# singhhp1069/charon

Measured on AMD Instinct MI355X. Metric: verified+aggregated 3-of-4 threshold BLS sigs/sec at 1/2/4/8 MI355X, higher is better.
Workload: dtype u32 (Fp 14x28-bit limbs); 1 GPU; config2: 3-of-4, 10000 DVs x 1 attestation per GPU; parallelism=shard1, inflight_launches=3, batches_per_launch=16, rlc_group=16, rlc_chunk=8, gident=0, subgroup_batch=0, level0=passed, hw_queues=4

## Files before the change

### charon_amd/_native.py

```python
from __future__ import annotations

import ctypes
import os
import shutil
import subprocess

PKG = os.path.dirname(os.path.abspath(__file__))
ROOT = os.path.dirname(PKG)
CSRC = os.path.join(PKG, "csrc")
LIB_PATH = os.path.join(PKG, "libtbls_gpu.so")
HEADER = os.path.join(ROOT, "include", "tbls_gpu.h")
HEADERS = [HEADER, os.path.join(ROOT, "include", "tbls_ssz.h")]


def _hipcc():
    for c in ("/opt/rocm/bin/hipcc", shutil.which("hipcc") or ""):
        if c and os.path.exists(c):
            return c
    raise RuntimeError("hipcc not found: cannot build libtbls_gpu.so")


def _clangxx():
    c = "/opt/rocm/llvm/bin/clang++"
    if not os.path.exists(c):
# ... 158 lines not shown
        ("slots", ctypes.c_uint32),
        ("verify_mode", ctypes.c_uint32),
        ("rlc_group", ctypes.c_uint32),
        ("rlc_seed", ctypes.c_uint64),
        ("rlc_chunk", ctypes.c_uint32),
        ("streams_per_slot", ctypes.c_uint32),
        ("rlc_batch", ctypes.c_uint32),
        ("gident", ctypes.c_uint32),
        ("fb_window", ctypes.c_uint32),
        ("subgroup_batch", ctypes.c_uint32),
        ("express_partials", ctypes.c_uint32),
        ("l0_duty_partials", ctypes.c_uint32),
        ("l0_msg_share", ctypes.c_uint32),
        ("sgb_tri_partials", ctypes.c_uint32),
        ("sgb_tri_m", ctypes.c_uint32),
    ]


SIGNATURES = {
    "tbg_init": (ctypes.c_int, [ctypes.POINTER(TbgConfig), ctypes.POINTER(ctypes.c_void_p)]),
    "tbg_destroy": (None, [ctypes.c_void_p]),
    "tbg_strerror": (ctypes.c_char_p, [ctypes.c_int]),
    "tbg_device_count": (ctypes.c_int, []),
    "tbg_device_cu_count": (ctypes.c_int, [ctypes.c_int]),
    "tbg_synchronize": (ctypes.c_int, [ctypes.c_void_p]),
    "tbg_load_pubkeys": (ctypes.c_int, [ctypes.c_void_p, ctypes.c_void_p, ctypes.c_uint32,
                                        ctypes.POINTER(ctypes.c_uint32), ctypes.c_void_p]),
    "tbg_pubkey_count": (ctypes.c_uint32, [ctypes.c_void_p]),
    "tbg_submit": (ctypes.c_int, [ctypes.c_void_p, ctypes.POINTER(TbgBatch), ctypes.POINTER(ctypes.c_uint64)]),
    "tbg_collect": (ctypes.c_int, [ctypes.c_void_p, ctypes.c_uint64, ctypes.c_void_p, ctypes.c_void_p,
# ... 79 lines not shown
```

### charon_amd/csrc/k_msm.hip

```cpp
#define TBG_ADD_DBL_INLINE 1
#ifndef TBG_SCHED_FENCE
#define TBG_SCHED_FENCE 1
#endif
#include "tbls_launch.h"
#include "bls_msm.h"
#include "bls_pair.h"
#include "bls_batchinv.h"

namespace tbg {

__global__ void __launch_bounds__(BINV_BLOCK) k_pubkey_tables(const G1A* pk, const G1A* xpk, const int32_t* status,
                                                              uint32_t n, G1A* tab) {
  const uint32_t i = blockIdx.x * blockDim.x + threadIdx.x;
  const bool in = i < n;
  const bool ok = in && status[i] == DEC_OK;
  G1A p0{fp_zero(), fp_zero()}, x0 = p0;
  if (ok) {
    p0 = pk[i];
    x0 = xpk[i];
  }
#pragma unroll 1
  for (int k = 0; k < (int)PK_TAB; ++k) {
    const G1J e = ok ? rlc_key_table_w2_entry(p0, x0, k) : jac_inf<Fp>();
    G1A a{fp_zero(), fp_zero()};
    const bool got = block_jac_to_aff<BINV_WAVES>(e, ok, a);
    if (in) tab[(size_t)PK_TAB * i + k] = got ? a : G1A{fp_zero(), fp_zero()};
  }
}

__global__ void TBG_LAUNCH k_rlc_g1_l0(DevBatch B, const G1A* tab, const int32_t* pk_status, uint32_t n_pk) {
  const uint32_t i = blockIdx.x * blockDim.x + threadIdx.x;
  if (i >= B.n_partials || B.partial_status[i] != TBG_PS_NOT_VERIFIED) return;
  const uint32_t pid = B.pubkey_ids[i];
  const bool fused = l0_fused(B);
  if (pid >= n_pk || pk_status[pid] != DEC_OK) {
    B.partial_status[i] = TBG_PS_ERR_PUBKEY;
    if (fused) B.counters[CNT_L0_BAD] = 1;
    return;
  }
  if (fused) {
    const uint4 v = *(const uint4*)(B.l0f_u + 4ull * i);
    const uint32_t uf[4] = {v.x, v.y, v.z, v.w};
    B.part_p[i] = rlc_mul_key_l0f(tab + (size_t)PK_TAB * pid, fp_from_const(G1_BETA), uf);
    return;
  }
  const uint64_t r = rlc_scalar(B.rlc_seed, i);
  uint32_t u[4];
  rlc_digits(r, u);
  B.msm_r[i] = r;
  B.part_p[i] = rlc_mul_key(tab + (size_t)PK_TAB * pid, u);
#pragma unroll
  for (int k = 0; k < 4; ++k) {
    bool neg;
    atomicAdd(&B.msm_off[msm_bucket(u[k], neg)], 1u);
  }
}

namespace l0duty {
static_assert(BINV_BLOCK == kBlock, "k_rlc_g1_l0: the workgroup of the batched inversion");
__global__ void TBG_LAUNCH k_rlc_g1_l0(DevBatch B, const G1A* tab, const int32_t* pk_status, uint32_t n_pk) {
  const uint32_t d = blockIdx.x * blockDim.x + threadIdx.x;
  const bool in = d < B.n_duties;
  uint32_t i0 = 0, n = 0, cand = 0;
  if (in) {
    i0 = B.duty_first[d];
    n = B.duty_first[d + 1] - i0;
    for (uint32_t k = 0; k < n; ++k) {
      const uint32_t i = i0 + k;
      if (B.partial_status[i] != TBG_PS_NOT_VERIFIED) continue;
      const uint32_t pid = B.pubkey_ids[i];
      if (pid >= n_pk || pk_status[pid] != DEC_OK) {
        B.partial_status[i] = TBG_PS_ERR_PUBKEY;
        B.counters[CNT_L0_BAD] = 1;
        continue;
      }
      ++cand;
// ... 171 lines not shown
  __shared__ Jac<Fp2x> lds[2 * PAIRS];
  if (B.counters[CNT_L0_BAD]) return;
  const uint32_t pr = threadIdx.x >> 1;
  Jac<Fp2x> acc = jac_add_in<Fp2x, true>(px_load(B.msm_sum[2 * pr]), px_load(B.msm_sum[2 * pr + 1]));
  acc = pair_tree_sum<PAIRS>(acc, lds);
  if (pr != 0) return;
  if (jac_is_inf(acc)) {
    if (pair_par() == 0) B.counters[CNT_L0_BAD] = 1;
    return;
  }
  const Fp2x zi = f_inv(acc.Z);
  const Fp2x zi2 = f_sqr(zi);
  px_store(*B.batch_pt, Aff<Fp2x>{f_mul(acc.X, zi2), f_mul(acc.Y, f_mul(zi2, zi))});
}

__global__ void __launch_bounds__(2 * L0F_PAIRS) k_l0f_reduce(DevBatch B, uint32_t n_sg, uint32_t wq, uint32_t n_t) {
  __shared__ Jac<Fp2x> lds[2 * L0F_PAIRS];
  if (B.counters[CNT_L0_BAD]) return;
  const uint32_t pr = threadIdx.x >> 1, b = blockIdx.x;
  const bool qcol = b < SGB_K * wq;
  const uint32_t col = qcol ? b / wq : SGB_K, chunk = qcol ? b % wq : b - SGB_K * wq;
  const uint32_t count = qcol ? n_sg : n_sg * n_t;
  const uint32_t a0 = chunk * L0F_CHUNK + pr * L0F_PER, a1 = min(a0 + L0F_PER, count);
  Jac<Fp2x> acc = jac_inf<Fp2x>();
#pragma unroll 1
  for (uint32_t a = a0; a < a1; ++a) {
    if (qcol) {
      acc = jac_add_in<Fp2x, true>(acc, px_load(B.sgb_part[sgb_q_slot(B, a, col)]));
    } else {
      acc = jac_add_in<Fp2x, true>(acc, px_load(B.sgb_t[a]));
    }
  }
  acc = pair_tree_sum<L0F_PAIRS>(acc, lds);
  if (pr == 0) px_store(B.l0f_sum[b], acc);
}

__global__ void __launch_bounds__(2 * L0F_PAIRS) k_l0f_fold(DevBatch B, uint32_t wq, uint32_t wt) {
  TBG_URGENT();
  __shared__ Jac<Fp2x> lds[2 * L0F_PAIRS];
  if (B.counters[CNT_L0_BAD]) return;
  const uint32_t pr = threadIdx.x >> 1, col = blockIdx.x;
  const uint32_t first = col < SGB_K ? col * wq : SGB_K * wq, count = col < SGB_K ? wq : wt;
  Jac<Fp2x> acc = jac_inf<Fp2x>();
#pragma unroll 1
  for (uint32_t a = pr; a < count; a += L0F_PAIRS) acc = jac_add_in<Fp2x, true>(acc, px_load(B.l0f_sum[first + a]));
  acc = pair_tree_sum<L0F_PAIRS>(acc, lds);
  if (pr == 0) px_store(B.l0f_sum[SGB_K * wq + wt + col], acc);
}

constexpr uint32_t L0F_HORNER_THREADS = 8;
__global__ void __launch_bounds__(64) k_l0f_horner(DevBatch B, uint32_t base) {
  TBG_URGENT();
  __shared__ Jac<Fp2x> lds[L0F_HORNER_THREADS];
  if (B.counters[CNT_L0_BAD]) return;
  const int j = (int)(threadIdx.x >> 1);
  const G2J* tot = B.l0f_sum + base;
  const int e0 = l0f_first(j), e1 = l0f_first(j + 1);
  Jac<Fp2x> acc = px_load(tot[e1 - 1]);
#pragma unroll 1
  for (int e = e1 - 2; e >= e0; --e) acc = l0f_mul13_add(acc, px_load(tot[e]));
  acc = l0f_term(acc, px_load(tot[SGB_K]), j);
// ... 2 lines not shown
  if (jac_is_inf(acc)) {
    if (pair_par() == 0) B.counters[CNT_L0_BAD] = 1;
    return;
  }
  const Fp2x zi = f_inv(acc.Z);
  const Fp2x zi2 = f_sqr(zi);
  px_store(*B.batch_pt, Aff<Fp2x>{f_mul(acc.X, zi2), f_mul(acc.Y, f_mul(zi2, zi))});
}

void launch_pubkey_tables(const G1A* pk, const G1A* xpk, const int32_t* status, uint32_t n, G1A* tab, hipStream_t st) {
  if (n) TBG_KLAUNCH(k_pubkey_tables, dim3((n + BINV_BLOCK - 1) / BINV_BLOCK), dim3(BINV_BLOCK), st, pk, xpk, status, n,
                     tab);
}

void launch_l0_keys(const DevBatch& B, const G1A* pk_tab, const int32_t* pk_status, uint32_t n_pk, hipStream_t st) {
  if (l0_per_duty(B)) {
    using l0duty::k_rlc_g1_l0;
    TBG_KLAUNCH(k_rlc_g1_l0, grid_for(B.n_duties), dim3(kBlock), st, B, pk_tab, pk_status, n_pk);
    return;
  }
  if (B.n_partials) TBG_KLAUNCH(k_rlc_g1_l0, grid_for(B.n_partials), dim3(kBlock), st, B, pk_tab, pk_status, n_pk);
}

void launch_l0_msm(const DevBatch& B, hipStream_t st) {
  TBG_KLAUNCH(k_msm_scan, dim3(1), dim3(kScanBlock), st, B);
  if (B.n_partials) TBG_KLAUNCH(k_msm_scatter, grid_for(B.n_partials), dim3(kBlock), st, B);
  TBG_KLAUNCH(k_msm_bucket_part, grid_for(2 * MSM_BUCKETS * MSM_SPLIT), dim3(kBlock), st, B);
  TBG_KLAUNCH(k_msm_bucket, grid_for(2 * MSM_BUCKETS), dim3(kBlock), st, B);
  TBG_KLAUNCH(k_msm_tree, dim3(MSM_TREE_WG), dim3(2 * MSM_TREE_PAIRS), st, B);
  TBG_KLAUNCH(k_msm_tree_final, dim3(1), dim3(MSM_TREE_WG), st, B);
}

void launch_l0_fused_s(const DevBatch& B, hipStream_t st) {
  const uint32_t n_sg = sgb_groups(B.n_partials, B.sgb_m), n_t = sgb_t_slices(B.sgb_m);
  const uint32_t wq = l0f_q_chunks(n_sg), wt = l0f_t_chunks(n_sg, B.sgb_m);
  TBG_KLAUNCH(k_l0f_reduce, dim3(SGB_K * wq + wt), dim3(2 * L0F_PAIRS), st, B, n_sg, wq, n_t);
  TBG_KLAUNCH(k_l0f_fold, dim3(L0F_COLS), dim3(2 * L0F_PAIRS), st, B, wq, wt);
  TBG_KLAUNCH(k_l0f_horner, dim3(1), dim3(L0F_HORNER_THREADS), st, B, SGB_K * wq + wt);
}

}
```

### charon_amd/csrc/k_rlc.hip

```cpp
#define TBG_ADD_DBL_INLINE 1
#ifndef TBG_SCHED_FENCE
#define TBG_SCHED_FENCE 1
#endif
#include "tbls_launch.h"
#include "bls_h2c.h"
#include "bls_lines.h"
#include "bls_hex.h"
#include "bls_rlc.h"
#include "bls_batchinv.h"
#include "bls_row.h"

namespace tbg {

__device__ __forceinline__ bool rlc_usable(const DevBatch& B, uint32_t i, const int32_t* pk_status, uint32_t n_pk) {
  int32_t st = B.partial_status[i];
  if (st != TBG_PS_NOT_VERIFIED && st != TBG_PS_ERR_PUBKEY) return false;
  uint32_t pid = B.pubkey_ids[i];
  return pid < n_pk && pk_status[pid] == DEC_OK;
}
__device__ __forceinline__ bool rlc_candidate(const DevBatch& B, uint32_t i) {
  return B.partial_status[i] == TBG_PS_NOT_VERIFIED;
}

__device__ __forceinline__ bool rlc_combinable(const DevBatch& B, uint32_t d) {
// ... 664 lines not shown
}

void launch_rlc_prepare(const DevBatch& B, const G1A* pk_aff, const G1A* pk_tab, const int32_t* pk_status,
                        uint32_t n_pk, hipStream_t st, void (*after_keys)(const DevBatch&, hipStream_t)) {
  if (B.sets) launch_set_init(B, st);
  if (!B.n_duties) return;
  if (B.rlc_group == 0) {
    if (B.n_partials) TBG_KLAUNCH(k_list_all_partials, grid_for(B.n_partials), dim3(kBlock), st, B, pk_status, n_pk);
    if (after_keys) after_keys(B, st);
    return;
  }
  uint32_t n_groups = (B.n_duties + B.rlc_group - 1) / B.rlc_group;
  if (B.rlc_batch) {
    launch_l0_keys(B, pk_tab, pk_status, n_pk, st);
    if (after_keys) after_keys(B, st);
    if (l0_fused(B)) launch_l0_fused_s(B, st);
    else launch_l0_msm(B, st);
    if (!l0_per_duty(B)) TBG_KLAUNCH(k_rlc_duty_sum<DSUM_L0_P>, duty_grid(B), dim3(BINV_BLOCK), st, B);
    if (l0_by_msg(B)) launch_l0m_sums(B, st);
    launch_l0_lines(B, st);
    return;
  }
  if (after_keys) after_keys(B, st);
  launch_rlc_g1(B, pk_tab, pk_aff, pk_status, n_pk, st);
  TBG_KLAUNCH(k_rlc_duty_sum<DSUM_P>, duty_grid(B), dim3(BINV_BLOCK), st, B);
  launch_gm_group_s(B, st);
  launch_lines_fold(B, FOLD_GROUPS, n_groups, st);
}

static void launch_narrowing(const DevBatch& B, const G1A* pk_aff, uint32_t n_groups, uint32_t nch, hipStream_t st) {
  TBG_KLAUNCH(k_rlc_resolve_groups, grid_for(B.n_duties), dim3(kBlock), st, B);
  launch_gm_failed_partials(B, pk_aff, st);
// ... 84 lines not shown
```

### charon_amd/csrc/tbls_engine.hip

```cpp
#include <hip/hip_runtime.h>
#include <cstdio>
#include <cstdlib>
#include <cstring>
#include <cmath>
#include <functional>
#include <algorithm>
#include <atomic>
#include <chrono>
#include <mutex>
#include <new>
#include <random>
#include <thread>
#include <vector>
#include "tbls_launch.h"
#include "bls_l0msg.h"
#include "bls_lines.h"

using namespace tbg;

namespace tbg {
void debug_after_launch(const char* kernel, hipStream_t st) {
  static const bool on = getenv("TBG_DEBUG_SYNC") && getenv("TBG_DEBUG_SYNC")[0] == '1';
  if (!on) return;
  hipEvent_t a;
// ... 88 lines not shown
  tbg_ticket next_ticket = 1;
  float last_ms[8] = {};
  uint32_t rlc_group = 16;
  uint32_t rlc_chunk = 4;
  bool chunk_auto = true;
  bool rlc_auto = false;
  uint32_t rlc_batch = TBG_RLC_L0_AUTO;
  double invalid_ema = 0.0;
  uint64_t rlc_seed = 0;
  uint64_t seed_ctr = 0;
  uint32_t gident = TBG_GIDENT_OFF;
  uint32_t fb_window = TBG_FB_WINDOW;
  uint32_t sgb_mode = TBG_SGB_AUTO;
  uint32_t express_max = TBG_EXPRESS_PARTIALS;
  uint32_t l0_duty_partials = TBG_L0_DUTY_PARTIALS;
  uint32_t l0_msg_share = TBG_L0_MSG_SHARE;
  uint32_t sgb_tri_partials = TBG_SGB_TRI_PARTIALS;
  uint32_t sgb_tri_m = SGB_TRI_M;
  uint32_t n_simd = 1024;
  std::atomic<uint64_t> host[8] = {};
  double nonsub_ema = 0.0;
};

#define HIP_TRY(x)                       \
  do {                                   \
    hipError_t e_ = (x);                 \
    if (e_ != hipSuccess) return TBG_E_DEVICE; \
  } while (0)

static size_t arena_size(size_t need) {
// ... 83 lines not shown
  if (cfg && cfg->rlc_chunk) {
    c->rlc_chunk = cfg->rlc_chunk;
    c->chunk_auto = false;
  }
  if (c->rlc_group > 4096 || c->rlc_chunk > 4096) { delete c; return TBG_E_INVALID_ARG; }
  if (cfg && cfg->rlc_batch > TBG_RLC_L0_OFF) { delete c; return TBG_E_INVALID_ARG; }
  if (cfg) c->rlc_batch = cfg->rlc_batch;
  c->rlc_seed = cfg ? cfg->rlc_seed : 0;
  if (cfg && cfg->gident > TBG_GIDENT_CHUNKS) { delete c; return TBG_E_INVALID_ARG; }
  c->gident = cfg ? cfg->gident : (uint32_t)TBG_GIDENT_OFF;
  if (cfg && cfg->fb_window) c->fb_window = cfg->fb_window;
  if (cfg && cfg->subgroup_batch > TBG_SGB_OFF) { delete c; return TBG_E_INVALID_ARG; }
  if (cfg) c->sgb_mode = cfg->subgroup_batch;
  if (cfg && cfg->express_partials) c->express_max = cfg->express_partials;
  if (cfg && cfg->l0_duty_partials) c->l0_duty_partials = cfg->l0_duty_partials;
  if (cfg && cfg->l0_msg_share) c->l0_msg_share = cfg->l0_msg_share;
  if (cfg && cfg->sgb_tri_partials) c->sgb_tri_partials = cfg->sgb_tri_partials;
  if (cfg && cfg->sgb_tri_m) c->sgb_tri_m = cfg->sgb_tri_m;
  if (!sgb_triple(c->sgb_tri_m) || c->sgb_tri_m > SGB_TRI_M_MAX || (c->sgb_tri_m & (c->sgb_tri_m - 1))) {
    delete c;
    return TBG_E_INVALID_ARG;
  }
  if (hipSetDevice(dev) != hipSuccess || hipStreamCreateWithFlags(&c->stream, hipStreamNonBlocking) != hipSuccess ||
      hipEventCreateWithFlags(&c->retire_ev, hipEventDisableTiming) != hipSuccess ||
      hipEventCreateWithFlags(&c->keys_ready, hipEventDisableTiming) != hipSuccess) {
    if (c->retire_ev) hipEventDestroy(c->retire_ev);
    if (c->stream) hipStreamDestroy(c->stream);
    delete c;
    return TBG_E_DEVICE;
  }
// ... 742 lines not shown
  B.gm_hist = (uint32_t*)(dw + w_gmhist);
  B.gm_order = (uint32_t*)(dw + w_gmorder);
  B.sgb = sgb ? 1u : 0u;
  B.sgb_m = sgb_m;
  B.sgb_split = sgb_split;
  B.sgb_off = (uint32_t*)(dw + w_sgoff);
  B.sgb_ent = (uint32_t*)(dw + w_sgent);
  B.sgb_part = (G2J*)(dw + w_sgpart);
  B.sgb_rank = (uint32_t*)(dw + w_sgrank);
  B.sgb_code = (uint32_t*)(dw + w_sgcode);
  B.sgb_bad = (uint32_t*)(dw + w_sgbad);
  B.sgb_t = (G2J*)(dw + w_sgt);
  B.l0f_sum = (G2J*)(dw + w_l0fsum);
  B.l0f_u = (uint32_t*)(dw + w_l0fu);
  B.l0_duty_partials = c->l0_duty_partials;
  B.l0_msg_share = l0m ? c->l0_msg_share : TBG_L0_MSG_NEVER;
  B.l0m_n_chunks = l0m ? parts[n_batches - 1].ch1 : 0;
  B.l0m_max_chunks = l0m ? parts[n_batches - 1].maxch : 0;
  B.msg_first = (const uint32_t*)(di + o_mfirst);
  B.msg_duty = (const uint32_t*)(di + o_mduty);
  B.l0m_chunk_first = (const uint32_t*)(di + o_cfirst);
  B.l0m_chunk_msg = (const uint32_t*)(di + o_cmsg);
  B.l0m_part = (G1J*)(dw + w_l0mpart);
  B.l0m_cnt = (uint32_t*)(dw + w_l0mcnt);
  B.l0m_q = (G1A*)(dw + w_l0mq);
  B.l0m_state = (int32_t*)(dw + w_l0mst);
  B.agg_acc = (G2J*)(dw + w_aacc);
  B.agg_list = (uint32_t*)(dw + w_alist);

  hipStream_t st = s->st;
// ... 721 lines not shown
```

### charon_amd/csrc/tbls_launch.h

```cpp
#pragma once
#include <hip/hip_runtime.h>
#include "bls_curve.h"
#include "bls_lines.h"
#include "../../include/tbls_gpu.h"

namespace tbg {

constexpr int kBlock = 64;
constexpr uint32_t PK_TAB = 8;
#ifndef TBG_FB_WINDOW
#define TBG_FB_WINDOW 32768u
#endif

#ifndef TBG_MIN_WAVES
#define TBG_MIN_WAVES 1
#endif
#define TBG_LAUNCH __launch_bounds__(64, TBG_MIN_WAVES)
#ifndef TBG_PAIR_WAVES
#define TBG_PAIR_WAVES 2
#endif
#ifndef TBG_DECODE_WAVES
#define TBG_DECODE_WAVES 2
#endif
#define TBG_LAUNCH_N(w) __launch_bounds__(64, w)
// ... 43 lines not shown
  G1A* cid_p;
  uint32_t* cid_lines;
  uint32_t gident;
  uint32_t* grp_fe;
  uint32_t* gid_list;
  G1A* gid_p;
  uint32_t* gid_lines;
  uint32_t* gid_f;
  uint32_t* id_fe;
  uint32_t* id_list;
  G1A* id_p;
  uint32_t fb_window, fb_base;
  uint32_t fb_full;
  uint32_t* id_lines;
  uint32_t rlc_batch;
  uint64_t* msm_r;
  uint32_t* msm_off;
  uint32_t* msm_cur;
  uint32_t* msm_ent;
  G2J* msm_part;
  G2J* msm_bkt;
  G2J* msm_sum;
  G2A* batch_pt;
  uint32_t* batch_lines;
  uint32_t* batch_f;
  uint32_t* grp_f;
  uint32_t* gm_off;
  uint32_t* gm_ent;
  G2J* gm_part;
  uint32_t* gm_lead;
// ... 23 lines not shown
  const uint32_t* l0m_chunk_msg;
  G1J* l0m_part;
  uint32_t* l0m_cnt;
  G1A* l0m_q;
  int32_t* l0m_state;
  G2J* agg_acc;
  uint32_t* agg_list;
  int32_t* partial_status;
  int32_t* duty_status;
  uint8_t* agg;
  uint32_t sets;
  uint32_t n_sets;
  const uint32_t* duty_set;
  int32_t* set_status;
};
enum SetTail : int { SET_BAD = 0, SET_ANY = 1, SET_TAIL = 2 };

enum RlcState : int32_t { RLC_NONE = 0, RLC_COMBINED = 1, RLC_EACH = 2 };
enum GroupState : int32_t { GRP_EMPTY = 0, GRP_LINES = 1, GRP_OK = 2, GRP_FAIL = 3, GRP_GID = 4,
                            GRP_BAD = 5 };
enum Counter : int { CNT_DUTIES = 0, CNT_PARTIALS = 1, CNT_AGG = 2, CNT_CHUNKS = 3, CNT_CID = 4, CNT_L0_BAD = 5,
                     CNT_L0_OK = 6, CNT_GID = 7, CNT_LAZY = 8, CNT_WORDS = 9 };

constexpr uint32_t MSM_BUCKETS = 32768;
constexpr uint32_t MSM_SPLIT = 4;
constexpr uint32_t MSM_SUM_ENTRIES = 128;
#ifndef TBG_SGB_M
#define TBG_SGB_M 1024
#endif
#ifndef TBG_SGB_SPLIT
#define TBG_SGB_SPLIT 4
#endif
constexpr uint32_t SGB_M = TBG_SGB_M;
constexpr uint32_t SGB_M_MIN = 64;
constexpr uint32_t SGB_K = 18;
constexpr uint32_t SGB_V = 6;
constexpr uint32_t SGB_BUCKETS = SGB_K * SGB_V;
// ... 28 lines not shown
TBG_HD uint32_t sgb_ent_stride(uint32_t m) {
  return m * (sgb_triple(m) ? SGB_TRIPLES : sgb_paired(m) ? SGB_PAIRS : SGB_K);
}
TBG_HD uint32_t sgb_rank_stride(uint32_t m) { return sgb_triple(m) ? SGB_TBUCKETS : sgb_paired(m) ? SGB_PBUCKETS : 0u; }
constexpr uint32_t SGB_TFOLD = SGB_TBUCKETS + SGB_TRIPLES * SGB_TF1;
TBG_HD uint32_t sgb_part_stride(uint32_t m) {
  return sgb_triple(m)   ? SGB_TFOLD + SGB_BUCKETS
         : sgb_paired(m) ? SGB_PBUCKETS + SGB_BUCKETS
                         : SGB_BUCKETS * sgb_split_for(m);
}
TBG_HD size_t sgb_q_slot(const DevBatch& B, uint32_t g, uint32_t k) {
  return (size_t)sgb_part_stride(B.sgb_m) * g + (sgb_triple(B.sgb_m)   ? SGB_TFOLD + SGB_V * k
                                                 : sgb_paired(B.sgb_m) ? SGB_PBUCKETS + SGB_V * k
                                                                       : SGB_V * k * B.sgb_split);
}
TBG_HD bool l0_fused(const DevBatch& B) {
  return B.rlc_batch && B.rlc_group && B.sgb && B.n_partials;
}
TBG_HD bool l0_per_duty(const DevBatch& B) { return l0_fused(B) && B.n_partials >= B.l0_duty_partials; }
TBG_HD bool l0_by_msg(const DevBatch& B) {
  return l0_fused(B) && B.l0_msg_share != TBG_L0_MSG_NEVER && (uint64_t)B.n_msgs * B.l0_msg_share <= B.n_duties;
}
constexpr uint32_t SGB_T_PER = 32;
TBG_HD uint32_t sgb_t_slices(uint32_t m) { return m / SGB_T_PER; }
constexpr uint32_t L0F_COLS = SGB_K + 1;
constexpr uint32_t L0F_PAIRS = 128, L0F_PER = 4;
constexpr uint32_t L0F_CHUNK = L0F_PAIRS * L0F_PER;
TBG_HD uint32_t l0f_q_chunks(uint32_t n_sg) { return (n_sg + L0F_CHUNK - 1) / L0F_CHUNK; }
TBG_HD uint32_t l0f_t_chunks(uint32_t n_sg, uint32_t m) { return (n_sg * sgb_t_slices(m) + L0F_CHUNK - 1) / L0F_CHUNK; }
TBG_HD uint32_t l0f_sum_entries(uint32_t n_sg, uint32_t m) {
  return SGB_K * l0f_q_chunks(n_sg) + l0f_t_chunks(n_sg, m) + L0F_COLS;
}
constexpr uint32_t L0_TREE_FAN = 4;
TBG_HD uint32_t grp_f_entries(uint32_t n_groups) { return n_groups + n_groups / (L0_TREE_FAN - 1) + 40; }
enum MillerMode : int { MILLER_GROUPS = 0, MILLER_L0 = 1, MILLER_GROUP_S = 2 };
enum DutySumPhase : int { DSUM_L0_P = 1, DSUM_FALLBACK_S = 2, DSUM_P = 3 };
constexpr uint32_t GM_W = 4, GM_V = 8, GM_BUCKETS = GM_W * GM_V;

constexpr uint32_t CHUNK_DEGENERATE = 0x80000000u;
constexpr uint32_t ID_DEGENERATE = 0x80000000u;
enum FoldKind : int { FOLD_GROUPS = 0, FOLD_CHUNKS = 1, FOLD_CID = 2, FOLD_IDENT = 3, FOLD_GID = 5 };

TBG_HD bool fb_in_pass(const DevBatch& B, uint32_t k) { return B.fb_window == 0 || k - B.fb_base < B.fb_window; }
TBG_HD size_t fb_slot(const DevBatch& B, uint32_t k) { return (size_t)LINES_WORDS * (k - B.fb_base); }
template <class F>
TBG_HD void fb_pass_loop(const DevBatch& B, uint32_t first, uint32_t stride, uint32_t count, F&& body) {
// ... 77 lines not shown
```

### charon_amd/engine.py

```python
from __future__ import annotations

import ctypes
import itertools
from dataclasses import dataclass

import numpy as np

from . import _native

PS_INVALID, PS_VALID, PS_NOT_VERIFIED = 0, 1, 2
PS_ERR_FLAGS, PS_ERR_FIELD, PS_ERR_CURVE, PS_ERR_SUBGROUP, PS_ERR_IDENTITY, PS_ERR_PUBKEY = -1, -2, -3, -4, -5, -6
DS_OK, DS_NOT_AGGREGATED = 0, 1
DS_INSUFFICIENT, DS_INSUFFICIENT_VALID = -20, -21
DS_AGG_TOO_FEW, DS_AGG_DUPLICATE_ID, DS_AGG_IDENTITY, DS_DECODE = -22, -23, -24, -25
SS_ERROR, SS_INVALID, SS_VALID = 30, 31, 32
OP_VERIFY, OP_AGGREGATE, OP_VERIFY_AGGREGATE = 1, 2, 3
NO_PUBKEY = 0xFFFFFFFF
TIMING_KEYS = ["decode", "hash", "combine", "h_lines", "verify", "lagrange", "aggregate", "total"]
VERIFY_RLC, VERIFY_EACH = 0, 1
RLC_L0_AUTO, RLC_L0_ON, RLC_L0_OFF = 0, 1, 2
GIDENT_OFF, GIDENT_L3, GIDENT_CHUNKS = 0, 1, 2
SGB_AUTO, SGB_ON, SGB_OFF = 0, 1, 2
SGB_SCHEDULES = ("none", "classic", "paired", "triple")
EXPRESS_OFF = 0xFFFFFFFF
L0_DUTY_ALWAYS, L0_DUTY_NEVER = 1, 0xFFFFFFFF
SGB_TRI_NEVER = 0xFFFFFFFF
L0_MSG_ALWAYS, L0_MSG_NEVER = 1, 0xFFFFFFFF
L0_NOT_RUN, L0_PASSED, L0_FAILED = 0, 1, 2
HOST_STAT_KEYS = ["submits", "partials_submitted", "pack_ns", "enqueue_ns", "collects", "partials_collected",
                  "gather_ns", "wait_ns"]
MULTI_HOST_STAT_KEYS = ["submits", "partials", "build_ns", "submit_wall_ns", "collects", "collect_wall_ns"] + \
    ["ctx_" + k for k in HOST_STAT_KEYS] + ["contexts", "reserved"]
E_PENDING = -6
E_INVALID_ARG, E_TICKET = -1, -7


class EngineError(RuntimeError):
    pass


# ... 40 lines not shown


def device_cu_count(device: int = 0) -> int:
    n = int(_native.load().tbg_device_cu_count(device))
    if n <= 0:
        raise EngineError(f"tbg_device_cu_count({device}): {_native.load().tbg_strerror(n).decode()} ({n})")
    return n


class Engine:

    def __init__(self, device: int = 0, slots: int = 3, verify_mode: int = VERIFY_RLC, rlc_group: int = 0,
                 rlc_seed: int = 0, rlc_chunk: int = 0, streams_per_slot: int = 0, rlc_batch: int = 0,
                 gident: int = GIDENT_OFF, fb_window: int = 0, subgroup_batch: int = SGB_AUTO,
                 express_partials: int = 0, l0_duty_partials: int = 0, l0_msg_share: int = 0,
                 sgb_tri_partials: int = 0, sgb_tri_m: int = 0):
        self._lib = _native.load()
        cfg = _native.TbgConfig(device=device, max_partials=0, max_duties=0, max_msg_bytes=0, slots=slots,
                                verify_mode=verify_mode, rlc_group=rlc_group, rlc_seed=rlc_seed,
                                rlc_chunk=rlc_chunk, streams_per_slot=streams_per_slot, rlc_batch=rlc_batch,
                                gident=gident, fb_window=fb_window, subgroup_batch=subgroup_batch,
                                express_partials=express_partials, l0_duty_partials=l0_duty_partials,
                                l0_msg_share=l0_msg_share, sgb_tri_partials=sgb_tri_partials, sgb_tri_m=sgb_tri_m)
        h = ctypes.c_void_p()
        rc = self._lib.tbg_init(ctypes.byref(cfg), ctypes.byref(h))
        self._check(rc, "tbg_init")
        self._h = h
        self.device = device
        self.uid = next(_serial)
        self._keep = {}

    def _check(self, rc, what):
        if rc != 0:
            raise EngineError(f"{what}: {self._lib.tbg_strerror(rc).decode()} ({rc})")

    def close(self):
        if getattr(self, "_h", None):
            self._lib.tbg_destroy(self._h)
# ... 376 lines not shown
```

### include/tbls_gpu.h

```cpp
#ifndef TBLS_GPU_H
#define TBLS_GPU_H

#include <stddef.h>
#include <stdint.h>

#ifdef __cplusplus
extern "C" {
#endif

#define TBG_OK 0
#define TBG_E_INVALID_ARG (-1)
#define TBG_E_DEVICE (-2)
#define TBG_E_OOM (-3)
#define TBG_E_NO_DEVICE (-4)
#define TBG_E_BUSY (-5)
#define TBG_E_PENDING (-6)
#define TBG_E_TICKET (-7)

#define TBG_PS_INVALID 0
#define TBG_PS_VALID 1
#define TBG_PS_NOT_VERIFIED 2
#define TBG_PS_ERR_FLAGS (-1)
#define TBG_PS_ERR_FIELD (-2)
#define TBG_PS_ERR_CURVE (-3)
// ... 36 lines not shown
  uint32_t slots;
  uint32_t verify_mode;
  uint32_t rlc_group;
  uint64_t rlc_seed;
  uint32_t rlc_chunk;
  uint32_t streams_per_slot;
  uint32_t rlc_batch;
  uint32_t gident;
  uint32_t fb_window;
  uint32_t subgroup_batch;
  uint32_t express_partials;
  uint32_t l0_duty_partials;
  uint32_t l0_msg_share;
  uint32_t sgb_tri_partials;
  uint32_t sgb_tri_m;
} tbg_config;
#define TBG_SGB_TRI_PARTIALS 262144u
#define TBG_SGB_TRI_NEVER 0xFFFFFFFFu
#define TBG_L0_MSG_SHARE 2u
#define TBG_L0_MSG_NEVER 0xFFFFFFFFu
#define TBG_L0_DUTY_PARTIALS 600000u
#define TBG_L0_DUTY_NEVER 0xFFFFFFFFu
#define TBG_EXPRESS_PARTIALS 4096u
#define TBG_EXPRESS_OFF 0xFFFFFFFFu
#define TBG_SGB_AUTO 0
#define TBG_SGB_ON 1
#define TBG_SGB_OFF 2
#define TBG_SGB_AUTO_MAX 2.5e-3
#define TBG_GIDENT_OFF 0
#define TBG_GIDENT_L3 1
#define TBG_GIDENT_CHUNKS 2
// ... 109 lines not shown
```

Before: 3.938 million DV-duties/s (n verifies + 1 aggregate each).

## Fuse level-0 G2 reduce/fold/horner tail into key kernel via atomic last-block chaining

Moves the three-kernel level-0 fused S reduction (reduce, fold, Horner) into extra leading blocks of the k_rlc_g1_l0 key kernel. The last-arriving block per column and overall is detected with agent-scope atomic counters and performs the fold and final Horner step. This removes two kernel launches and their serialization on the stream, at the cost of smaller chunking (kBlock/2 pairs), extra counters, and a larger key-kernel grid. It is gated by a threshold of 131072 partials.

After: 4.018 million DV-duties/s (n verifies + 1 aggregate each), median of 6. 1.02x the previous value.

```diff
diff --git a/charon_amd/_native.py b/charon_amd/_native.py
--- a/charon_amd/_native.py
+++ b/charon_amd/_native.py
@@ -196,6 +196,7 @@
         ("l0_msg_share", ctypes.c_uint32),
         ("sgb_tri_partials", ctypes.c_uint32),
         ("sgb_tri_m", ctypes.c_uint32),
+        ("l0_tail_partials", ctypes.c_uint32),
     ]
 
 
diff --git a/charon_amd/csrc/bls_l0tail.h b/charon_amd/csrc/bls_l0tail.h
--- /dev/null
+++ b/charon_amd/csrc/bls_l0tail.h
@@ -0,0 +1,73 @@
+#pragma once
+#include "bls_rlc.h"
+#include "bls_pair.h"
+
+namespace tbg {
+
+constexpr uint32_t L0T_QCOLS = 18;
+constexpr uint32_t L0T_COLS = L0T_QCOLS + 1;
+constexpr uint32_t L0T_PAIRS = 32, L0T_PER = 4;
+constexpr uint32_t L0T_CHUNK = L0T_PAIRS * L0T_PER;
+
+struct L0tShape { uint32_t n_sg, n_t, wq, wt; };
+TBG_HD uint32_t l0t_chunks(uint32_t points) { return (points + L0T_CHUNK - 1) / L0T_CHUNK; }
+TBG_HD L0tShape l0t_shape(uint32_t n_sg, uint32_t n_t) { return {n_sg, n_t, l0t_chunks(n_sg), l0t_chunks(n_sg * n_t)}; }
+TBG_HD uint32_t l0t_blocks(const L0tShape& s) { return L0T_QCOLS * s.wq + s.wt; }
+TBG_HD uint32_t l0t_sum_entries(const L0tShape& s) { return l0t_blocks(s) + L0T_COLS; }
+
+template <class F>
+TBG_HD Jac<F> l0t_mul13_add(const Jac<F>& acc, const Jac<F>& q) {
+  Jac<F> t = jac_add(jac_dbl(acc), acc);
+  t = jac_add(jac_dbl(jac_dbl(t)), acc);
+  return jac_add(t, q);
+}
+template <class F>
+TBG_HD Jac<F> l0t_term(const Jac<F>& A, const Jac<F>& T, int j) {
+  Jac<F> r = jac_add(jac_dbl(A), T);
+  for (int k = 0; k < j; ++k) r = g2_psi_g(r);
+  return r;
+}
+
+template <class Env>
+TBG_HD void l0t_block(Env& env, const L0tShape& sh, uint32_t b) {
+  using F = typename Env::F;
+  using P = Jac<F>;
+  const bool qcol = b < L0T_QCOLS * sh.wq;
+  const uint32_t col = qcol ? b / sh.wq : L0T_QCOLS, chunk = qcol ? b % sh.wq : b - L0T_QCOLS * sh.wq;
+  const uint32_t count = qcol ? sh.n_sg : sh.n_sg * sh.n_t;
+  typename Env::V v = env.per_pair(L0T_PAIRS, [&](uint32_t pr) {
+    const uint32_t a0 = chunk * L0T_CHUNK + pr * L0T_PER;
+    P acc = jac_inf<F>();
+#pragma unroll 1
+    for (uint32_t a = a0; a < a0 + L0T_PER && a < count; ++a)
+      acc = jac_add(acc, qcol ? env.load_q(a, col) : env.load_t(a));
+    return acc;
+  });
+  env.store_sum(b, env.tree(v, L0T_PAIRS));
+  const uint32_t n_chunks = qcol ? sh.wq : sh.wt;
+  if (env.arrive_col(col) != n_chunks - 1) return;
+
+  env.acquire();
+  const uint32_t first = qcol ? col * sh.wq : L0T_QCOLS * sh.wq;
+  v = env.per_pair(L0T_PAIRS, [&](uint32_t pr) {
+    P acc = jac_inf<F>();
+#pragma unroll 1
+    for (uint32_t a = pr; a < n_chunks; a += L0T_PAIRS) acc = jac_add(acc, env.load_sum(first + a));
+    return acc;
+  });
+  const uint32_t tot = l0t_blocks(sh);
+  env.store_sum(tot + col, env.tree(v, L0T_PAIRS));
+  if (env.arrive_done() != L0T_COLS - 1) return;
+
+  env.acquire();
+  v = env.per_pair(4, [&](uint32_t j) {
+    const int e0 = l0f_first((int)j), e1 = l0f_first((int)j + 1);
+    P acc = env.load_sum(tot + (uint32_t)e1 - 1);
+#pragma unroll 1
+    for (int e = e1 - 2; e >= e0; --e) acc = l0t_mul13_add(acc, env.load_sum(tot + (uint32_t)e));
+    return l0t_term(acc, env.load_sum(tot + L0T_QCOLS), (int)j);
+  });
+  env.finish(env.tree(v, 4));
+}
+
+}
diff --git a/charon_amd/csrc/k_msm.hip b/charon_amd/csrc/k_msm.hip
--- a/charon_amd/csrc/k_msm.hip
+++ b/charon_amd/csrc/k_msm.hip
@@ -6,8 +6,93 @@
 #include "bls_msm.h"
 #include "bls_pair.h"
 #include "bls_batchinv.h"
+#include "bls_l0tail.h"
 
 namespace tbg {
+
+static_assert(L0T_QCOLS == SGB_K && L0T_COLS == L0F_COLS && L0T_PAIRS == L0F_PAIRS && L0T_PER == L0F_PER,
+              "bls_l0tail.h: the chunking of tbls_launch.h");
+struct L0tDev {
+  using F = Fp2x;
+  using V = Jac<Fp2x>;
+  const G2J* sgb_part;
+  const G2J* sgb_t;
+  G2J* sum;
+  uint32_t* counters;
+  G2A* batch_pt;
+  uint32_t sgb_m, sgb_split;
+  Jac<Fp2x>* lds;
+
+  template <class Fn>
+  TBG_DEV V per_pair(uint32_t n, Fn&& f) const {
+    const uint32_t pr = threadIdx.x >> 1;
+    V acc = jac_inf<Fp2x>();
+    if (pr < n) acc = f(pr);
+    return acc;
+  }
+  TBG_DEV V tree(V acc, uint32_t n) const {
+    const uint32_t t = threadIdx.x, pr = t >> 1;
+#pragma unroll 1
+    for (uint32_t s = 1; s < n; s <<= 1) {
+      lds[t] = acc;
+      __syncthreads();
+      if ((pr & (2 * s - 1)) == 0 && pr + s < n) {
+        const V o = lds[t + 2 * s];
+        acc = jac_add(acc, o);
+      }
+      __syncthreads();
+    }
+    return acc;
+  }
+  TBG_DEV V load_q(uint32_t g, uint32_t col) const { return px_load(sgb_part[sgb_q_slot(sgb_m, sgb_split, g, col)]); }
+  TBG_DEV V load_t(uint32_t a) const { return px_load(sgb_t[a]); }
+  TBG_DEV V load_sum(uint32_t i) const { return px_load(sum[i]); }
+  TBG_DEV void store_sum(uint32_t i, const V& p) const {
+    if ((threadIdx.x >> 1) == 0) px_store(sum[i], p);
+  }
+  TBG_DEV uint32_t arrive(uint32_t* counter) const {
+    __asm__ __volatile__("s_waitcnt vmcnt(0)" ::: "memory");
+    uint32_t ticket = 0;
+    if (threadIdx.x == 0) {
+      __builtin_amdgcn_fence(__ATOMIC_RELEASE, "agent");
+      __asm__ __volatile__("s_waitcnt vmcnt(0)" ::: "memory");
+      ticket = __hip_atomic_fetch_add((__attribute__((address_space(1))) uint32_t*)counter, 1u, __ATOMIC_RELAXED,
+                                      __HIP_MEMORY_SCOPE_AGENT);
+    }
+    return (uint32_t)__builtin_amdgcn_readfirstlane((int)ticket);
+  }
+  TBG_DEV uint32_t arrive_col(uint32_t col) const { return arrive(counters + CNT_L0F_COL + col); }
+  TBG_DEV uint32_t arrive_done() const { return arrive(counters + CNT_L0F_DONE); }
+  TBG_DEV void acquire() const {
+    __builtin_amdgcn_fence(__ATOMIC_ACQUIRE, "agent");
+    __asm__ __volatile__("s_waitcnt vmcnt(0)" ::: "memory");
+    __syncthreads();
+  }
+  TBG_DEV void finish(const V& S) const {
+    if ((threadIdx.x >> 1) != 0) return;
+    if (jac_is_inf(S)) {
+      if (pair_par() == 0) counters[CNT_L0_BAD] = 1;
+      return;
+    }
+    const Fp2x zi = f_inv(S.Z);
+    const Fp2x zi2 = f_sqr(zi);
+    px_store(*batch_pt, Aff<Fp2x>{f_mul(S.X, zi2), f_mul(S.Y, f_mul(zi2, zi))});
+  }
+};
+
+__device__ __noinline__ void l0f_s_role(const G2J* sgb_part, const G2J* sgb_t, G2J* sum, uint32_t* counters,
+                                        G2A* batch_pt, uint32_t sgb_m, uint32_t sgb_split, uint32_t n_sg) {
+  __shared__ Jac<Fp2x> lds[kBlock];
+  L0tDev env{sgb_part, sgb_t, sum, counters, batch_pt, sgb_m, sgb_split, lds};
+  l0t_block(env, l0t_shape(n_sg, sgb_t_slices(sgb_m)), blockIdx.x);
+}
+TBG_DEV bool l0f_s_block(const DevBatch& B, uint32_t n_s) {
+  if (blockIdx.x >= n_s) return false;
+  TBG_URGENT();
+  l0f_s_role(B.sgb_part, B.sgb_t, B.l0f_sum, B.counters, B.batch_pt, B.sgb_m, B.sgb_split,
+             sgb_groups(B.n_partials, B.sgb_m));
+  return true;
+}
 
 __global__ void __launch_bounds__(BINV_BLOCK) k_pubkey_tables(const G1A* pk, const G1A* xpk, const int32_t* status,
                                                               uint32_t n, G1A* tab) {
@@ -28,8 +113,10 @@
   }
 }
 
-__global__ void TBG_LAUNCH k_rlc_g1_l0(DevBatch B, const G1A* tab, const int32_t* pk_status, uint32_t n_pk) {
-  const uint32_t i = blockIdx.x * blockDim.x + threadIdx.x;
+__global__ void TBG_LAUNCH_N(TBG_PAIR_WAVES) k_rlc_g1_l0(DevBatch B, const G1A* tab, const int32_t* pk_status,
+                                                          uint32_t n_pk, uint32_t n_s) {
+  if (l0f_s_block(B, n_s)) return;
+  const uint32_t i = (blockIdx.x - n_s) * blockDim.x + threadIdx.x;
   if (i >= B.n_partials || B.partial_status[i] != TBG_PS_NOT_VERIFIED) return;
   const uint32_t pid = B.pubkey_ids[i];
   const bool fused = l0_fused(B);
@@ -58,8 +145,10 @@
 
 namespace l0duty {
 static_assert(BINV_BLOCK == kBlock, "k_rlc_g1_l0: the workgroup of the batched inversion");
-__global__ void TBG_LAUNCH k_rlc_g1_l0(DevBatch B, const G1A* tab, const int32_t* pk_status, uint32_t n_pk) {
-  const uint32_t d = blockIdx.x * blockDim.x + threadIdx.x;
+__global__ void TBG_LAUNCH_N(TBG_PAIR_WAVES) k_rlc_g1_l0(DevBatch B, const G1A* tab, const int32_t* pk_status,
+                                                          uint32_t n_pk, uint32_t n_s) {
+  if (l0f_s_block(B, n_s)) return;
+  const uint32_t d = (blockIdx.x - n_s) * blockDim.x + threadIdx.x;
   const bool in = d < B.n_duties;
   uint32_t i0 = 0, n = 0, cand = 0;
   if (in) {
@@ -261,14 +350,14 @@
   px_store(*B.batch_pt, Aff<Fp2x>{f_mul(acc.X, zi2), f_mul(acc.Y, f_mul(zi2, zi))});
 }
 
-__global__ void __launch_bounds__(2 * L0F_PAIRS) k_l0f_reduce(DevBatch B, uint32_t n_sg, uint32_t wq, uint32_t n_t) {
-  __shared__ Jac<Fp2x> lds[2 * L0F_PAIRS];
+__global__ void __launch_bounds__(2 * L0FK_PAIRS) k_l0f_reduce(DevBatch B, uint32_t n_sg, uint32_t wq, uint32_t n_t) {
+  __shared__ Jac<Fp2x> lds[2 * L0FK_PAIRS];
   if (B.counters[CNT_L0_BAD]) return;
   const uint32_t pr = threadIdx.x >> 1, b = blockIdx.x;
   const bool qcol = b < SGB_K * wq;
   const uint32_t col = qcol ? b / wq : SGB_K, chunk = qcol ? b % wq : b - SGB_K * wq;
   const uint32_t count = qcol ? n_sg : n_sg * n_t;
-  const uint32_t a0 = chunk * L0F_CHUNK + pr * L0F_PER, a1 = min(a0 + L0F_PER, count);
+  const uint32_t a0 = chunk * L0FK_CHUNK + pr * L0FK_PER, a1 = min(a0 + L0FK_PER, count);
   Jac<Fp2x> acc = jac_inf<Fp2x>();
 #pragma unroll 1
   for (uint32_t a = a0; a < a1; ++a) {
@@ -278,20 +367,20 @@
       acc = jac_add_in<Fp2x, true>(acc, px_load(B.sgb_t[a]));
     }
   }
-  acc = pair_tree_sum<L0F_PAIRS>(acc, lds);
+  acc = pair_tree_sum<L0FK_PAIRS>(acc, lds);
   if (pr == 0) px_store(B.l0f_sum[b], acc);
 }
 
-__global__ void __launch_bounds__(2 * L0F_PAIRS) k_l0f_fold(DevBatch B, uint32_t wq, uint32_t wt) {
-  TBG_URGENT();
-  __shared__ Jac<Fp2x> lds[2 * L0F_PAIRS];
+__global__ void __launch_bounds__(2 * L0FK_PAIRS) k_l0f_fold(DevBatch B, uint32_t wq, uint32_t wt) {
+  TBG_URGENT();
+  __shared__ Jac<Fp2x> lds[2 * L0FK_PAIRS];
   if (B.counters[CNT_L0_BAD]) return;
   const uint32_t pr = threadIdx.x >> 1, col = blockIdx.x;
   const uint32_t first = col < SGB_K ? col * wq : SGB_K * wq, count = col < SGB_K ? wq : wt;
   Jac<Fp2x> acc = jac_inf<Fp2x>();
 #pragma unroll 1
-  for (uint32_t a = pr; a < count; a += L0F_PAIRS) acc = jac_add_in<Fp2x, true>(acc, px_load(B.l0f_sum[first + a]));
-  acc = pair_tree_sum<L0F_PAIRS>(acc, lds);
+  for (uint32_t a = pr; a < count; a += L0FK_PAIRS) acc = jac_add_in<Fp2x, true>(acc, px_load(B.l0f_sum[first + a]));
+  acc = pair_tree_sum<L0FK_PAIRS>(acc, lds);
   if (pr == 0) px_store(B.l0f_sum[SGB_K * wq + wt + col], acc);
 }
 
@@ -324,12 +413,14 @@
 }
 
 void launch_l0_keys(const DevBatch& B, const G1A* pk_tab, const int32_t* pk_status, uint32_t n_pk, hipStream_t st) {
+  const uint32_t n_s = l0_tail(B) ? l0f_s_blocks(B) : 0u;
   if (l0_per_duty(B)) {
     using l0duty::k_rlc_g1_l0;
-    TBG_KLAUNCH(k_rlc_g1_l0, grid_for(B.n_duties), dim3(kBlock), st, B, pk_tab, pk_status, n_pk);
-    return;
-  }
-  if (B.n_partials) TBG_KLAUNCH(k_rlc_g1_l0, grid_for(B.n_partials), dim3(kBlock), st, B, pk_tab, pk_status, n_pk);
+    TBG_KLAUNCH(k_rlc_g1_l0, dim3(n_s + grid_for(B.n_duties).x), dim3(kBlock), st, B, pk_tab, pk_status, n_pk, n_s);
+    return;
+  }
+  if (B.n_partials)
+    TBG_KLAUNCH(k_rlc_g1_l0, dim3(n_s + grid_for(B.n_partials).x), dim3(kBlock), st, B, pk_tab, pk_status, n_pk, n_s);
 }
 
 void launch_l0_msm(const DevBatch& B, hipStream_t st) {
@@ -343,9 +434,9 @@
 
 void launch_l0_fused_s(const DevBatch& B, hipStream_t st) {
   const uint32_t n_sg = sgb_groups(B.n_partials, B.sgb_m), n_t = sgb_t_slices(B.sgb_m);
-  const uint32_t wq = l0f_q_chunks(n_sg), wt = l0f_t_chunks(n_sg, B.sgb_m);
-  TBG_KLAUNCH(k_l0f_reduce, dim3(SGB_K * wq + wt), dim3(2 * L0F_PAIRS), st, B, n_sg, wq, n_t);
-  TBG_KLAUNCH(k_l0f_fold, dim3(L0F_COLS), dim3(2 * L0F_PAIRS), st, B, wq, wt);
+  const uint32_t wq = l0fk_q_chunks(n_sg), wt = l0fk_t_chunks(n_sg, B.sgb_m);
+  TBG_KLAUNCH(k_l0f_reduce, dim3(SGB_K * wq + wt), dim3(2 * L0FK_PAIRS), st, B, n_sg, wq, n_t);
+  TBG_KLAUNCH(k_l0f_fold, dim3(L0F_COLS), dim3(2 * L0FK_PAIRS), st, B, wq, wt);
   TBG_KLAUNCH(k_l0f_horner, dim3(1), dim3(L0F_HORNER_THREADS), st, B, SGB_K * wq + wt);
 }
 
diff --git a/charon_amd/csrc/k_rlc.hip b/charon_amd/csrc/k_rlc.hip
--- a/charon_amd/csrc/k_rlc.hip
+++ b/charon_amd/csrc/k_rlc.hip
@@ -702,8 +702,8 @@
   if (B.rlc_batch) {
     launch_l0_keys(B, pk_tab, pk_status, n_pk, st);
     if (after_keys) after_keys(B, st);
-    if (l0_fused(B)) launch_l0_fused_s(B, st);
-    else launch_l0_msm(B, st);
+    if (!l0_fused(B)) launch_l0_msm(B, st);
+    else if (!l0_tail(B)) launch_l0_fused_s(B, st);
     if (!l0_per_duty(B)) TBG_KLAUNCH(k_rlc_duty_sum<DSUM_L0_P>, duty_grid(B), dim3(BINV_BLOCK), st, B);
     if (l0_by_msg(B)) launch_l0m_sums(B, st);
     launch_l0_lines(B, st);
diff --git a/charon_amd/csrc/tbls_engine.hip b/charon_amd/csrc/tbls_engine.hip
--- a/charon_amd/csrc/tbls_engine.hip
+++ b/charon_amd/csrc/tbls_engine.hip
@@ -126,6 +126,7 @@
   uint32_t sgb_mode = TBG_SGB_AUTO;
   uint32_t express_max = TBG_EXPRESS_PARTIALS;
   uint32_t l0_duty_partials = TBG_L0_DUTY_PARTIALS;
+  uint32_t l0_tail_partials = TBG_L0_TAIL_PARTIALS;
   uint32_t l0_msg_share = TBG_L0_MSG_SHARE;
   uint32_t sgb_tri_partials = TBG_SGB_TRI_PARTIALS;
   uint32_t sgb_tri_m = SGB_TRI_M;
@@ -239,6 +240,7 @@
   if (cfg) c->sgb_mode = cfg->subgroup_batch;
   if (cfg && cfg->express_partials) c->express_max = cfg->express_partials;
   if (cfg && cfg->l0_duty_partials) c->l0_duty_partials = cfg->l0_duty_partials;
+  if (cfg && cfg->l0_tail_partials) c->l0_tail_partials = cfg->l0_tail_partials;
   if (cfg && cfg->l0_msg_share) c->l0_msg_share = cfg->l0_msg_share;
   if (cfg && cfg->sgb_tri_partials) c->sgb_tri_partials = cfg->sgb_tri_partials;
   if (cfg && cfg->sgb_tri_m) c->sgb_tri_m = cfg->sgb_tri_m;
@@ -1011,6 +1013,7 @@
   B.l0f_sum = (G2J*)(dw + w_l0fsum);
   B.l0f_u = (uint32_t*)(dw + w_l0fu);
   B.l0_duty_partials = c->l0_duty_partials;
+  B.l0_tail_partials = c->l0_tail_partials;
   B.l0_msg_share = l0m ? c->l0_msg_share : TBG_L0_MSG_NEVER;
   B.l0m_n_chunks = l0m ? parts[n_batches - 1].ch1 : 0;
   B.l0m_max_chunks = l0m ? parts[n_batches - 1].maxch : 0;
diff --git a/charon_amd/csrc/tbls_launch.h b/charon_amd/csrc/tbls_launch.h
--- a/charon_amd/csrc/tbls_launch.h
+++ b/charon_amd/csrc/tbls_launch.h
@@ -81,6 +81,7 @@
   uint32_t fb_full;
   uint32_t* id_lines;
   uint32_t rlc_batch;
+  uint32_t l0_tail_partials;
   uint64_t* msm_r;
   uint32_t* msm_off;
   uint32_t* msm_cur;
@@ -134,13 +135,15 @@
   const uint32_t* duty_set;
   int32_t* set_status;
 };
+static_assert(offsetof(DevBatch, msm_r) == offsetof(DevBatch, rlc_batch) + 8, "l0_tail_partials fills rlc_batch's padding");
 enum SetTail : int { SET_BAD = 0, SET_ANY = 1, SET_TAIL = 2 };
 
 enum RlcState : int32_t { RLC_NONE = 0, RLC_COMBINED = 1, RLC_EACH = 2 };
 enum GroupState : int32_t { GRP_EMPTY = 0, GRP_LINES = 1, GRP_OK = 2, GRP_FAIL = 3, GRP_GID = 4,
                             GRP_BAD = 5 };
 enum Counter : int { CNT_DUTIES = 0, CNT_PARTIALS = 1, CNT_AGG = 2, CNT_CHUNKS = 3, CNT_CID = 4, CNT_L0_BAD = 5,
-                     CNT_L0_OK = 6, CNT_GID = 7, CNT_LAZY = 8, CNT_WORDS = 9 };
+                     CNT_L0_OK = 6, CNT_GID = 7, CNT_LAZY = 8,
+                     CNT_L0F_COL = 9, CNT_L0F_DONE = CNT_L0F_COL + 19, CNT_WORDS = CNT_L0F_DONE + 1 };
 
 constexpr uint32_t MSM_BUCKETS = 32768;
 constexpr uint32_t MSM_SPLIT = 4;
@@ -199,6 +202,11 @@
                                                  : sgb_paired(B.sgb_m) ? SGB_PBUCKETS + SGB_V * k
                                                                        : SGB_V * k * B.sgb_split);
 }
+TBG_HD size_t sgb_q_slot(uint32_t m, uint32_t split, uint32_t g, uint32_t k) {
+  return (size_t)sgb_part_stride(m) * g + (sgb_triple(m)   ? SGB_TFOLD + SGB_V * k
+                                           : sgb_paired(m) ? SGB_PBUCKETS + SGB_V * k
+                                                           : SGB_V * k * split);
+}
 TBG_HD bool l0_fused(const DevBatch& B) {
   return B.rlc_batch && B.rlc_group && B.sgb && B.n_partials;
 }
@@ -209,12 +217,23 @@
 constexpr uint32_t SGB_T_PER = 32;
 TBG_HD uint32_t sgb_t_slices(uint32_t m) { return m / SGB_T_PER; }
 constexpr uint32_t L0F_COLS = SGB_K + 1;
-constexpr uint32_t L0F_PAIRS = 128, L0F_PER = 4;
+constexpr uint32_t L0F_PAIRS = kBlock / 2, L0F_PER = 4;
 constexpr uint32_t L0F_CHUNK = L0F_PAIRS * L0F_PER;
+constexpr uint32_t L0FK_PAIRS = 128, L0FK_PER = 4;
+constexpr uint32_t L0FK_CHUNK = L0FK_PAIRS * L0FK_PER;
+static_assert(L0FK_CHUNK >= L0F_CHUNK, "l0f_sum holds either chunking");
+TBG_HD uint32_t l0fk_q_chunks(uint32_t n_sg) { return (n_sg + L0FK_CHUNK - 1) / L0FK_CHUNK; }
+TBG_HD uint32_t l0fk_t_chunks(uint32_t n_sg, uint32_t m) { return (n_sg * sgb_t_slices(m) + L0FK_CHUNK - 1) / L0FK_CHUNK; }
+static_assert(CNT_L0F_DONE - CNT_L0F_COL == (int)L0F_COLS, "one counter per column");
 TBG_HD uint32_t l0f_q_chunks(uint32_t n_sg) { return (n_sg + L0F_CHUNK - 1) / L0F_CHUNK; }
 TBG_HD uint32_t l0f_t_chunks(uint32_t n_sg, uint32_t m) { return (n_sg * sgb_t_slices(m) + L0F_CHUNK - 1) / L0F_CHUNK; }
 TBG_HD uint32_t l0f_sum_entries(uint32_t n_sg, uint32_t m) {
   return SGB_K * l0f_q_chunks(n_sg) + l0f_t_chunks(n_sg, m) + L0F_COLS;
+}
+TBG_HD bool l0_tail(const DevBatch& B) { return l0_fused(B) && B.n_partials >= B.l0_tail_partials; }
+TBG_HD uint32_t l0f_s_blocks(const DevBatch& B) {
+  const uint32_t n_sg = sgb_groups(B.n_partials, B.sgb_m);
+  return SGB_K * l0f_q_chunks(n_sg) + l0f_t_chunks(n_sg, B.sgb_m);
 }
 constexpr uint32_t L0_TREE_FAN = 4;
 TBG_HD uint32_t grp_f_entries(uint32_t n_groups) { return n_groups + n_groups / (L0_TREE_FAN - 1) + 40; }
diff --git a/charon_amd/engine.py b/charon_amd/engine.py
--- a/charon_amd/engine.py
+++ b/charon_amd/engine.py
@@ -24,6 +24,7 @@
 SGB_SCHEDULES = ("none", "classic", "paired", "triple")
 EXPRESS_OFF = 0xFFFFFFFF
 L0_DUTY_ALWAYS, L0_DUTY_NEVER = 1, 0xFFFFFFFF
+L0_TAIL_ALWAYS, L0_TAIL_NEVER = 1, 0xFFFFFFFF
 SGB_TRI_NEVER = 0xFFFFFFFF
 L0_MSG_ALWAYS, L0_MSG_NEVER = 1, 0xFFFFFFFF
 L0_NOT_RUN, L0_PASSED, L0_FAILED = 0, 1, 2
@@ -94,14 +95,15 @@
                  rlc_seed: int = 0, rlc_chunk: int = 0, streams_per_slot: int = 0, rlc_batch: int = 0,
                  gident: int = GIDENT_OFF, fb_window: int = 0, subgroup_batch: int = SGB_AUTO,
                  express_partials: int = 0, l0_duty_partials: int = 0, l0_msg_share: int = 0,
-                 sgb_tri_partials: int = 0, sgb_tri_m: int = 0):
+                 sgb_tri_partials: int = 0, sgb_tri_m: int = 0, l0_tail_partials: int = 0):
         self._lib = _native.load()
         cfg = _native.TbgConfig(device=device, max_partials=0, max_duties=0, max_msg_bytes=0, slots=slots,
                                 verify_mode=verify_mode, rlc_group=rlc_group, rlc_seed=rlc_seed,
                                 rlc_chunk=rlc_chunk, streams_per_slot=streams_per_slot, rlc_batch=rlc_batch,
                                 gident=gident, fb_window=fb_window, subgroup_batch=subgroup_batch,
                                 express_partials=express_partials, l0_duty_partials=l0_duty_partials,
-                                l0_msg_share=l0_msg_share, sgb_tri_partials=sgb_tri_partials, sgb_tri_m=sgb_tri_m)
+                                l0_msg_share=l0_msg_share, sgb_tri_partials=sgb_tri_partials, sgb_tri_m=sgb_tri_m,
+                                l0_tail_partials=l0_tail_partials)
         h = ctypes.c_void_p()
         rc = self._lib.tbg_init(ctypes.byref(cfg), ctypes.byref(h))
         self._check(rc, "tbg_init")
diff --git a/include/tbls_gpu.h b/include/tbls_gpu.h
--- a/include/tbls_gpu.h
+++ b/include/tbls_gpu.h
@@ -74,7 +74,10 @@
   uint32_t l0_msg_share;
   uint32_t sgb_tri_partials;
   uint32_t sgb_tri_m;
+  uint32_t l0_tail_partials;
 } tbg_config;
+#define TBG_L0_TAIL_PARTIALS 131072u
+#define TBG_L0_TAIL_NEVER 0xFFFFFFFFu
 #define TBG_SGB_TRI_PARTIALS 262144u
 #define TBG_SGB_TRI_NEVER 0xFFFFFFFFu
 #define TBG_L0_MSG_SHARE 2u
```
